# jthorborg/signalizer

Hardware: AMD Instinct MI355X
Metric: 32768-pt stereo STFT frames/sec (75% overlap); achieved HBM GB/s vs peak (higher is better)
Workload: dtype f32

## Files before the change

signalizer_amd/build.py:

```python
from __future__ import annotations

import os
import subprocess
import sys

HERE = os.path.dirname(os.path.abspath(__file__))
CSRC = os.path.join(HERE, "csrc")
LIB = os.path.join(HERE, "libsgz.so")
SOURCES = ["plan.cpp", "spectrum_fft.hip", "spectrum_real.hip", "spectrum_generic.hip", "spectrum_post.hip", "resonator.hip", "scope_vector.hip", "scope_dense.hip", "scope_stream.hip", "vector_stream.hip", "sharded.hip", "tracker.hip", "api.hip", "realtime.hip", "line_graph.hip", "view_translate.hip", "image_resize.hip", "ring_resize.hip", "spectrum_present.hip", "pcm.hip", "overview.hip", "overview_stats.hip", "overview_power.hip", "overview_cross.hip", "overview_flux.hip", "overview_pct.hip", "wave_columns.hip", "level_columns.hip", "truepeak_columns.hip", "loudness_columns.hip", "field_columns.hip", "band_columns.hip", "hist_columns.hip", "run_columns.hip"]
DRIVER = os.path.join(HERE, "librtdriver.so")
DRIVER_SRC = os.path.join(os.path.dirname(HERE), "tools", "rt_driver.cpp")
HEADERS = ["plan.hpp", "rt_lockfree.hpp", "kernels.hpp", "fft_common.hpp", "fft_scalar.hpp", "chunk_map.hpp", "real_common.hpp", "late_fix.hpp", "stft_body.hpp", "complex_dc.hpp", "decay_body.hpp", "runtime.hpp", "rt_common.hpp", "trace.hpp", "fade_chain.hpp", "scope_ring.hpp", "order_key.hpp", "column_lanes.hpp", "overview_kinds.hpp", os.path.join("..", "..", "include", "sgz.h")]


def _hipcc() -> str:
    for c in (os.environ.get("HIPCC"), "/opt/rocm/bin/hipcc", "hipcc"):
        if c and (os.path.isabs(c) and os.path.exists(c) or not os.path.isabs(c)):
            return c
    return "hipcc"


def stale() -> bool:
    if not os.path.exists(LIB):
        return True
# ... 7 lines not shown
        return LIB
    srcs = [os.path.join(CSRC, f) for f in SOURCES if os.path.exists(os.path.join(CSRC, f))]
    objs = []
    os.makedirs(os.path.join(HERE, "build"), exist_ok=True)
    procs = []
    for s in srcs:
        o = os.path.join(HERE, "build", os.path.basename(s) + ".o")
        objs.append(o)
        if s.endswith(".cpp"):
            cmd = [_hipcc(), "-O2", "-std=c++17", "-fPIC", "-ffp-contract=off", "-x", "c++", "-c", s, "-o", o]
        else:
            cmd = [_hipcc(), "--offload-arch=gfx950", "-O3", "-std=c++17", "-fPIC", "-fhip-fp32-correctly-rounded-divide-sqrt",
                   "-x", "hip", "-c", s, "-o", o] + os.environ.get("SGZ_EXTRA_HIPCC_FLAGS", "").split()
            if s.endswith(("spectrum_fft.hip", "spectrum_real.hip", "resonator.hip")):
                cmd.append("-fno-slp-vectorize")
        if verbose:
            print(" ".join(cmd))
        procs.append((s, subprocess.Popen(cmd, stdout=subprocess.PIPE, stderr=subprocess.STDOUT)))
    for s, p in procs:
        out, _ = p.communicate()
        if p.returncode != 0:
            sys.stderr.write(out.decode(errors="replace"))
            raise RuntimeError(f"hipcc failed on {s}")
    cmd = [_hipcc(), "--offload-arch=gfx950", "-shared", "-fPIC", "-o", LIB] + objs + ["-ldl"]
    subprocess.check_call(cmd)
    build_driver()
    return LIB



# ... 15 lines not shown
```

signalizer_amd/csrc/real_common.hpp:

```cpp
#pragma once
#include "chunk_map.hpp"
#include "fft_scalar.hpp"

namespace sgz {

struct ChannelIndex {
    int n, off;
    __device__ __forceinline__ int size() const { return n; }
    __device__ __forceinline__ int operator()(int k) const { return chunkPos(k - off); }
    __device__ __forceinline__ bool holds(int k) const { return k >= off && k <= off + n / 2; }
};

constexpr int realXFloats(int M) { return (chunkPos(M) + 1 + 16 + 1) & ~1; }

constexpr int kTw2Row = 34 * 2, kTw2Floats = 32 * kTw2Row;
constexpr size_t realExtraFloats(uint32_t maxSlots, uint32_t T, bool tw2InLds)
{
    const size_t a = size_t(maxSlots) + 1 + T, b = tw2InLds ? kTw2Floats + 4 : 0;
    return a > b ? a : b;
}

__device__ __forceinline__ float realBinMag(v2 a, v2 b, v2 w)
{
    const float ex = a.x + b.x, ey = a.y - b.y;
    const float dx = a.x - b.x, dy = a.y + b.y;
    const float xr = ex + (w.x * dy + w.y * dx);
    const float xi = ey + (w.y * dy - w.x * dx);
    return __builtin_amdgcn_sqrtf(xr * xr + xi * xi);
}

struct UnitId { int side, pair; uint32_t task, frame, self; };
template <bool MONO, typename P>
__device__ __forceinline__ UnitId unitOfIndex(const P &prm, uint32_t unit, const uint32_t nb, const bool mates = false)
{
    const uint32_t rs = prm.roundSize;
    if (nb >= 64u && rs >= 8u && (rs & 7u) == 0u) {
        const uint32_t base = (unit / rs) * rs;
        const uint32_t nbr = nb - base < rs ? nb - base : rs;
        const uint32_t x = (unit - base) & 7u;
        uint32_t i = (unit - base) >> 3;
        const uint32_t per = nbr >> 3, extra = nbr & 7u;
        if (mates) {
            const uint32_t c = rs >> 4, n = per + (x < extra ? 1u : 0u);
            if ((rs & 15u) == 0u && n > c && n <= 2u * c) {
                const uint32_t k = n - c;
                i = i < k ? 2u * i : i >= c ? 2u * (i - c) + 1u : i + k;
            }
        }
        unit = base + x * per + (x < extra ? x : extra) + i;
    }
    UnitId u;
    u.side = MONO ? 0 : int(unit & 1u);
    uint32_t task = MONO ? unit : unit >> 1;
    u.frame = task; u.pair = 0;
    if (prm.C > 1u) { const uint32_t F = uint32_t(prm.frames), pr = task / F, fr = task - pr * F; task = fr * prm.C + pr; u.frame = fr; u.pair = int(pr); }
    u.task = task;
    u.self = (task << 1) | uint32_t(u.side);
    return u;
}

template <bool MONO>
__device__ __forceinline__ UnitId unitOf(const RealParams &prm) { return unitOfIndex<MONO>(prm, blockIdx.x, gridDim.x); }

typedef const RealParams __attribute__((address_space(4))) WalkParams;
__device__ __forceinline__ WalkParams *walkParams()
{
    WalkParams *p = (WalkParams *)__builtin_amdgcn_kernarg_segment_ptr();
    asm volatile("" : "+s"(p));
    return p;
}
template <bool WALK> struct ParamsOf {
    typedef const RealParams T;
    static __device__ __forceinline__ T *get(const RealParams &launch) { return &launch; }
};
template <> struct ParamsOf<true> {
    typedef WalkParams T;
    static __device__ __forceinline__ T *get(const RealParams &) { return walkParams(); }
};

inline hipError_t grantLds(const void *kernel, size_t need, size_t (&granted)[64])
{
    int dev = 0;
    hipError_t e = hipGetDevice(&dev);
    if (e != hipSuccess) return e;
    if (dev >= 0 && dev < 64 && granted[dev] >= need) return hipSuccess;
    e = hipFuncSetAttribute(kernel, hipFuncAttributeMaxDynamicSharedMemorySize, int(need));
    if (e == hipSuccess && dev >= 0 && dev < 64) granted[dev] = need;
    return e;
}

}
```

signalizer_amd/csrc/spectrum_post.hip:

```cpp
#include <hip/hip_runtime.h>
#include <stdint.h>

#include <type_traits>

#include "decay_body.hpp"

namespace sgz {

__global__ void __launch_bounds__(256) decayLocalKernel(const DecayParams prm)
{
    const size_t perChunk = size_t(prm.C) * prm.sides * prm.P;
    const size_t gid = size_t(blockIdx.x) * blockDim.x + threadIdx.x;
    if (gid >= perChunk * prm.numChunks) return;
    const uint32_t chunk = uint32_t(gid / perChunk);
    const size_t rem = gid - size_t(chunk) * perChunk;
    const uint32_t pixel = uint32_t(rem % prm.P);
    const uint32_t ps = uint32_t(rem / prm.P);
    const uint32_t pair = ps / prm.sides, side = ps - pair * prm.sides;

    float a[G];
#pragma unroll
    for (int k = 0; k < G; ++k) {
        const size_t si = ((size_t(pair) * G + k) * prm.P + pixel) * 2 + side;
        a[k] = (chunk == 0 && prm.stateIn) ? prm.stateIn[si] : 0.f;
// ... 138 lines not shown
{
    for (;;) {
        uint32_t seen;
        asm volatile("ds_read_b32 %0, %1\n\ts_waitcnt lgkmcnt(0)" : "=v"(seen) : "v"(progressAddr) : "memory");
        if (seen >= chunk) break;
        __builtin_amdgcn_s_sleep(1);
    }
}

__device__ __forceinline__ uint32_t pixelGroup()
{
    const uint32_t b = blockIdx.x, n = gridDim.x;
    return (n & 7u) == 0 ? (b & 7u) * (n >> 3) + (b >> 3) : b;
}

template <int PX>
__global__ void __launch_bounds__(1024) decayColourFusedKernel(const DecayParams prm)
{
    __shared__ float aggS[kFusedChunks][PX];
    __shared__ float carryS[kFusedChunks][PX];
    __shared__ float magS[kFusedChunks * kMaxChunk][PX];
    __shared__ uint32_t progress;
    __shared__ double logTab[16][2];
    stageLogfTable(logTab);
    const uint32_t progressAddr = uint32_t(uintptr_t((__attribute__((address_space(3))) const void *)&progress));
    if (threadIdx.x == 0) progress = 0;
    const uint32_t tid = threadIdx.x;
    const size_t perFrame = size_t(prm.C) * prm.sides * prm.P;
    const float pole = prm.sc.pole[0];
    const uint32_t items = uint32_t(prm.frames) * PX;
    {
        constexpr int ROUNDS = kFusedChunks * kMaxChunk * PX / 1024;
        float m[ROUNDS], nyRe[ROUNDS], nyIm[ROUNDS], best[ROUNDS];
        const bool lateGroup = prm.hasLate && pixelGroup() * PX + PX > prm.late.fixFrom0;
#pragma unroll
        for (int r = 0; r < ROUNDS; ++r) {
            const uint32_t e = tid + 1024u * r, px = e % PX, f = e / PX;
            const uint32_t pixel = pixelGroup() * PX + px;
            const bool in = e < items && pixel < prm.P;
            m[r] = in ? prm.mapped[size_t(f) * perFrame + pixel] : 0.f;
            nyRe[r] = nyIm[r] = 0.f; best[r] = __builtin_inff();
            if (lateGroup && in && pixel >= prm.late.fixFrom0) {
                nyRe[r] = prm.late.ny[2 * size_t(f)]; nyIm[r] = prm.late.ny[2 * size_t(f) + 1];
                best[r] = lateBestSquare(prm.late, long(f), 0, pixel);
            }
        }
#pragma unroll
        for (int r = 0; r < ROUNDS; ++r) {
            const uint32_t e = tid + 1024u * r, px = e % PX, f = e / PX;
            const uint32_t pixel = pixelGroup() * PX + px;
            float v = m[r] * prm.magScale;
            if (lateGroup && e < items && pixel >= prm.late.fixFrom0 && pixel < prm.P)
                v = lateNyquistPixel(prm.late, lateNyquistValue(prm.late, nyRe[r], nyIm[r]), best[r], v);
            magS[f][px] = v;
        }
    }
    __syncthreads();
    static_assert(64 % PX == 0 && 960 % PX == 0, "thread tid's items tid - 64 + 960 k are all of pixel tid % PX");
    const uint32_t px = tid % PX;
    const uint32_t pixel = pixelGroup() * PX + px;
    if (tid < kFusedChunks * PX) {
// ... 565 lines not shown
    }
    if (prm.rgba && live && pl < len) reinterpret_cast<uchar4 *>(prm.rgba)[size_t(f0 + pl) * prm.P + pixel] = toRgba8(cb);
}

hipError_t launchDecayEmit(const DecayParams &prm, hipStream_t stream)
{
    const uint32_t firstChunk = (prm.rgba || prm.lines) ? 0u : prm.numChunks - 1;
    const unsigned grid = unsigned(size_t((prm.P + 31) / 32) * (prm.numChunks - firstChunk));
    static_assert(kMaxChunk == 8, "decayEmitPairsKernel: 8 frames x 32 pixels = one workgroup");
    if (prm.C >= 2) hipLaunchKernelGGL(decayEmitPairsKernel, dim3(grid), dim3(256), 0, stream, prm, firstChunk);
    else hipLaunchKernelGGL(decayEmitKernel, dim3(grid), dim3(256), 0, stream, prm, firstChunk);
    return hipGetLastError();
}

}
```

signalizer_amd/csrc/spectrum_real.hip:

```cpp
#include <algorithm>

#include "real_common.hpp"

#ifdef SGZ_DEBUG
#define RCLK(slot)                                                                                                     \
    do {                                                                                                               \
        if (prm.phaseClock && (tid & 63) == 0 && unit == long(prm.clkUnit)) prm.phaseClock[16 * (tid >> 6) + (slot)] = __builtin_readcyclecounter(); \
    } while (0)
#define RTRACE(which)                                                                                                  \
    do {                                                                                                               \
        if (prm.phaseClock && prm.clkUnit == 0xffffu && tid == 0) {                                                    \
            unsigned long long *t = prm.phaseClock + 256 + 4 * unit;                                                   \
            t[which] = __builtin_amdgcn_s_memrealtime();                                                               \
            if (which == 0) { t[2] = __builtin_amdgcn_s_getreg(4 | (31 << 11)); t[3] = __builtin_amdgcn_s_getreg(20 | (31 << 11)) | (static_cast<unsigned long long>(blockIdx.x) << 32); } \
        }                                                                                                              \
    } while (0)
#else
#define RCLK(slot) do { } while (0)
#define RTRACE(which) do { } while (0)
#endif

namespace sgz {

template <int R1, int LR1, int BASE, int Q = 0>
__device__ __forceinline__ void e1WriteRun(uint32_t wa, const v2 (&c)[32])
{
    if constexpr (Q < R1) { ldsWrite64<(Q & 15) * 512 * 8>(wa + uint32_t(Q >> 4) * 65536u, c[BASE + brev(Q, LR1)]); e1WriteRun<R1, LR1, BASE, Q + 1>(wa, c); }
}

template <int R1, int LR1, int Q = 0>
__device__ __forceinline__ void e1WritePairRun(uint32_t wa, const v2 (&c)[32])
{
    if constexpr (Q < R1) { ldsWrite128<(Q & 15) * 512 * 8>(wa + uint32_t(Q >> 4) * 65536u, c[brev(Q, LR1)], c[R1 + brev(Q, LR1)]); e1WritePairRun<R1, LR1, Q + 1>(wa, c); }
}
// ... 26 lines not shown

__device__ __forceinline__ void windowPairCos(v2 &lo, v2 &hi, const int a32, const v2 pc, const v2 ps, const v2 p0)
{
    v2 t = pc;
    if (a32 != 0) {
        const v2 k = v2{cos32(a32), sin32(a32)};
        v2 m;
        asm("v_pk_mul_f32 %0, %1, %2 op_sel:[0,1] op_sel_hi:[1,1]" : "=v"(m) : "v"(ps), "s"(k));
        asm("v_pk_fma_f32 %0, %1, %2, %3 op_sel:[0,0,0] op_sel_hi:[1,0,1] neg_lo:[0,0,1] neg_hi:[0,0,1]" : "=v"(t) : "v"(pc), "s"(k), "v"(m));
    }
    v2 wa, wb;
    asm("v_pk_add_f32 %0, %1, %2" : "=v"(wa) : "v"(t), "s"(p0));
    asm("v_pk_add_f32 %0, %1, %2 neg_lo:[1,0] neg_hi:[1,0]" : "=v"(wb) : "v"(t), "s"(p0));
    lo = lo * wa;
    hi = hi * wb;
}

template <int LR1, int MIX, typename P>
__device__ __forceinline__ void realMapSettle(const P &prm, float *lds, const int tid, const int side, const long task, const long self,
                                              const ChunkTables &tb, ChunkMap<(1 << (LR1 + 5))> &mapper, float *re, float *ce, float *spec)
{
    constexpr int R = 32, R1 = 1 << LR1, T = R1 * R, M = R1 * R * R, N = 2 * M;
    constexpr bool MONO = MIX == 1 || MIX == 3;
    const ChannelIndex at{N, side ? M : 0};
    [[maybe_unused]] const long unit = MONO ? task : self;
    if (prm.binsOut) {
        float *dst = prm.binsOut + size_t(task) * (N + 1) + (side ? M : 0);
        for (int i = tid; i <= M; i += T)
            if (MONO || i != (side ? 0 : M)) dst[i] = lds[chunkPos(i)];
    }
// ... 10 lines not shown
                out[x] = complexDcPixel(prm.recsFull[x], prm.weights, prm.invSize, N, prm.mode,
                                        [&](int k) { return k >= N ? 0.f : lds[chunkPos(k)]; },
                                        [&](int sl) { return make_float2(spec[2 * sl], spec[2 * sl + 1]); });
            }
        }
        return;
    }
}

[[maybe_unused]] __device__ __forceinline__ void setWavePriority(const uint32_t p)
{
    if (p != 0u) { if (p == 1u) __builtin_amdgcn_s_setprio(1); else if (p == 2u) __builtin_amdgcn_s_setprio(2); else __builtin_amdgcn_s_setprio(3); }
}

constexpr uint32_t kNyHopRows = 4;
template <int LR1, bool PRIO, bool SHARE>
__device__ __forceinline__ void nyquistUnit(const RealParams &prm, float *lds, const uint32_t light, const int tid)
{
    constexpr int LR = 5, R = 32, R1 = 1 << LR1, RR = R * R;
    static_assert(LR1 == 4, "the Nyquist workgroups mirror the two-columns-per-thread form (N = 32768)");
    [[maybe_unused]] const long unit = 2 * long(light) + 1;
    RTRACE(0);
#ifdef SGZ_IMAGE_PRIO
    if constexpr (PRIO) setWavePriority(prm.prioNy);
#endif
#ifdef SGZ_SCHED_SWEEP
    for (uint32_t k = 0; k < prm.nyDelay; ++k) __builtin_amdgcn_s_sleep(16);
#endif
    const uint32_t F = prm.nyFrames, perPair = uint32_t(prm.frames) / F + (uint32_t(prm.frames) % F != 0u);
    const uint32_t pair = light / perPair, f0 = (light - pair * perPair) * F;
    const uint32_t f1 = f0 + F < uint32_t(prm.frames) ? f0 + F : uint32_t(prm.frames);
    const float *X0 = prm.planar + size_t(2 * pair + 1) * prm.chStride;
    const uint32_t lane16 = uint32_t(tid) * 16u;
    const float4 ph[2] = {ldg(prm.winPhase, lane16 * 2u), ldg(prm.winPhase + 1, lane16 * 2u)};
    const v2 p0 = v2{prm.winP0, prm.winP0};
    v2 *lds2 = reinterpret_cast<v2 *>(lds);
    auto columnSum = [&](v2 (&c)[R1], const int u) {
        const v2 pc = v2{ph[u].x, ph[u].y}, ps = v2{ph[u].z, ph[u].w};
#pragma unroll
        for (int j = 0; j < R1 / 2; ++j) windowPairCos(c[j], c[j + R1 / 2], j * (32 / R1), pc, ps, p0);
        ditPacked<LR1, 0>(c);
        lds2[2 * tid + u] = c[0];
    };
    auto tree2 = [&]() {
        if (tid < R) {
            v2 s[R];
#pragma unroll
            for (int h = 0; h < R; ++h) s[h] = lds2[tid + R * h];
            ditPacked<LR, 0>(s);
            lds2[RR + tid] = s[0];
        }
    };
    auto tree3 = [&](const uint32_t f) {
        if (tid == 0) {
            v2 s[R];
#pragma unroll
            for (int r = 0; r < R; ++r) s[r] = lds2[RR + r];
            const float4 *tab = prm.tw2Full;
#pragma unroll
            for (int i = 0; i < R / 4; ++i) {
                const float4 wa = tab[i], wb = tab[i + R / 4];
                if (i == 0) bflyPackedFusedTw<true>(s[0], s[R / 2], v2{1.f, 0.f}, v2{wb.x, wb.y});
                else bflyPackedFusedTw<false>(s[2 * i], s[2 * i + R / 2], v2{wa.x, wa.y}, v2{wb.x, wb.y});
                bflyPackedFusedTw<false>(s[2 * i + 1], s[2 * i + 1 + R / 2], v2{wa.z, wa.w}, v2{wb.z, wb.w});
            }
            ditPacked<LR, 0, R, 2>(s);
            prm.ny[((size_t(f) * prm.C + pair) << 1) | 1u] = 2.f * (s[0].x - s[0].y);
        }
    };
    constexpr uint32_t HOPROWS = kNyHopRows;
    if (SHARE && f1 - f0 > 1u && prm.hop == HOPROWS * 2u * uint32_t(RR)) {
        typedef float v4 __attribute__((ext_vector_type(4)));
        v4 raw[R1];
        {
            const float *X = X0 + size_t(f0) * prm.hop;
#pragma unroll
            for (int j = 0; j < R1; ++j) raw[j] = ldgPinned<v4>(X, uint32_t(RR * j) * 8u, lane16);
        }
        for (uint32_t f = f0; f < f1; ++f) {
#pragma unroll
            for (int u = 0; u < 2; ++u) {
                v2 c[R1];
#pragma unroll
                for (int j = 0; j < R1; ++j) c[j] = u ? v2{raw[j].z, raw[j].w} : v2{raw[j].x, raw[j].y};
                columnSum(c, u);
            }
            if (f + 1u < f1) {
                const float *X = X0 + size_t(f + 1u) * prm.hop;
#pragma unroll
                for (int j = 0; j < R1 - int(HOPROWS); ++j) raw[j] = raw[j + int(HOPROWS)];
#pragma unroll
                for (int j = R1 - int(HOPROWS); j < R1; ++j) raw[j] = ldgPinned<v4>(X, uint32_t(RR * j) * 8u, lane16);
            }
            constexpr int PARK = R1 - int(HOPROWS);
            v4 *park = reinterpret_cast<v4 *>(lds + 4 * RR) + (tid & 63);
            if (__builtin_amdgcn_readfirstlane(tid) < 64) {
                __syncthreads();
#pragma unroll
                for (int j = 0; j < PARK; ++j) park[64 * j] = raw[j];
                tree2();
                __syncthreads();
                tree3(f);
#pragma unroll
                for (int j = 0; j < PARK; ++j) raw[j] = park[64 * j];
            } else {
                __syncthreads();
                __syncthreads();
            }
        }
        RTRACE(1);
        return;
    }
    for (uint32_t f = f0; f < f1; ++f) {
        const float *X = X0 + size_t(f) * prm.hop;
#pragma unroll
        for (int u = 0; u < 2; ++u) {
            v2 c[R1];
#pragma unroll
            for (int j = 0; j < R1; ++j) c[j] = ldgPinned<v2>(X, uint32_t(RR * j) * 8u + 8u * u, lane16);
            columnSum(c, u);
        }
        __syncthreads();
        tree2();
        __syncthreads();
        tree3(f);
    }
    RTRACE(1);
}

template <int LR1, bool WCOS, int MIX = 0, bool PRIO = false>
__global__ void __launch_bounds__(1 << (LR1 + 5), 4) stftRealKernel(const RealParams launchPrm)
{
    constexpr int LR = 5, R = 32, R1 = 1 << LR1, T = R1 * R, RR = R * R, M = R1 * RR, N = 2 * M, U = R / R1;
    constexpr bool MONO = MIX == 1 || MIX == 3;
    constexpr bool SIDE0 = MIX == 4;
    constexpr bool mixed = MIX == 2 || MIX == 3;
    constexpr int PADSTRIDE = chunkPos(T);
    constexpr int ROW = R + 2, TILE = R * ROW;
    constexpr int XFLOATS = realXFloats(M);
    static_assert((T / R) * TILE <= XFLOATS, "the exchange-2 tiles end below the twiddle table");
    constexpr int TAB = (XFLOATS + 3) & ~3;
    extern __shared__ __attribute__((aligned(16))) float lds[];
    const int tid0 = threadIdx.x;

    constexpr bool WALK = LR1 == 5 && MIX == 0 && WCOS;
    const uint32_t heavyUnits = SIDE0 ? uint32_t(launchPrm.frames) * launchPrm.C : gridDim.x;
    if constexpr (SIDE0) {
        if (blockIdx.x >= heavyUnits) { nyquistUnit<LR1, PRIO, PRIO>(launchPrm, lds, blockIdx.x - heavyUnits, opaque(tid0)); return; }
    }
    const uint32_t totalUnits = WALK ? uint32_t(launchPrm.frames) * launchPrm.C * 2u : heavyUnits;
    uint32_t walkIndex = blockIdx.x;
    UnitId uid = unitOfIndex<MONO || SIDE0>(launchPrm, walkIndex, totalUnits, SIDE0 && launchPrm.mateAdjacent != 0u);
    [[maybe_unused]] bool firstUnit = true;
    [[maybe_unused]] uint32_t prioEarly = 0u, prioLate = 0u, prioEnds = 0u;
    if constexpr (LR1 == 4) {
        const uint32_t cus = launchPrm.roundSize >> 1;
#ifndef SGZ_STAGGER
#define SGZ_STAGGER 5
#endif
        if (cus && !launchPrm.pipelined && gridDim.x >= 2u * cus && blockIdx.x >= cus && blockIdx.x < 2u * cus) {
#pragma unroll
            for (int k = 0; k < SGZ_STAGGER; ++k) __builtin_amdgcn_s_sleep(32);
        }
#ifdef SGZ_SCHED_SWEEP
        else if (SIDE0 && blockIdx.x >= cus) {
            for (uint32_t k = 0; k < launchPrm.mateDelay; ++k) __builtin_amdgcn_s_sleep(16);
        }
#endif
#ifndef SGZ_NO_PRIO
        if (cus && !launchPrm.pipelined && gridDim.x > 2u * cus && gridDim.x <= 3u * cus) {
#else
        if (false) {
#endif
            const uint32_t generation = blockIdx.x / cus;
            if (generation == 0u) __builtin_amdgcn_s_setprio(2); else if (generation == 1u) __builtin_amdgcn_s_setprio(1); else __builtin_amdgcn_s_setprio(3);
        }
#ifdef SGZ_IMAGE_PRIO
        if constexpr (PRIO) {
#ifdef SGZ_SCHED_SWEEP
            const uint32_t rolePrio = blockIdx.x >= cus ? launchPrm.prioMate : blockIdx.x + cus < heavyUnits ? launchPrm.prioFirst : 0u;
            const uint32_t scope = launchPrm.prioScope;
#else
            const uint32_t rolePrio = blockIdx.x >= cus ? (launchPrm.prioMate ? uint32_t(SGZ_PRIO_MATE) : 0u)
                                                        : blockIdx.x + cus < heavyUnits ? (launchPrm.prioFirst ? uint32_t(SGZ_PRIO_FIRST) : 0u) : 0u;
            constexpr uint32_t scope = SGZ_PRIO_SCOPE;
#endif
            prioEarly = (scope == 0u || scope == 3u) ? rolePrio : 0u;
            prioLate = (scope == 1u || scope == 2u) ? rolePrio : 0u;
            prioEnds = (scope & 1u) ? rolePrio : 0u;
            prioEarly = __builtin_amdgcn_readfirstlane(prioEarly); prioLate = __builtin_amdgcn_readfirstlane(prioLate); prioEnds = __builtin_amdgcn_readfirstlane(prioEnds);
        }
#endif
    }
    constexpr bool PAIRED = U == 2;
    constexpr int COLSTEP = PAIRED ? 1 : T, COLLANE = PAIRED ? 2 : 1;
    constexpr bool FRONT = LR1 >= 4 && !mixed && WCOS;
#ifdef SGZ_DIET
    constexpr bool DIET = PAIRED && FRONT && LR1 == 4;
#else
    constexpr bool DIET = false;
#endif
    constexpr bool STREAM = LR1 == 4 && PAIRED && FRONT && !DIET;
    [[maybe_unused]] float4 phase[U];
    [[maybe_unused]] float2 twA[U], twB[U];
    [[maybe_unused]] float4 tw2piece, tw2tail;
    v2 c[R];
    for (;;) {
    typename ParamsOf<WALK>::T &prm = *ParamsOf<WALK>::get(launchPrm);
    auto samplesOf = [&](const UnitId &u) {
        const int firstCh = MONO ? (prm.mode == SGZ_CH_RIGHT ? 1 : 0) : (mixed ? 0 : u.side);
        return prm.planar + size_t(2 * u.pair + firstCh) * prm.chStride + size_t(u.frame) * prm.hop;
    };
    auto elemOf = [&](int e) { const int u = e / R1, j = e % R1; return (PAIRED ? u : T * u) + RR * j; };
    auto requestSamples = [&](const float *X, const int tid, auto partTag) {
        constexpr int part = decltype(partTag)::value;
        const uint32_t lane8 = uint32_t(tid) * (PAIRED ? 16u : 8u);
        if constexpr (PAIRED) {
            typedef float v4 __attribute__((ext_vector_type(4)));
#pragma unroll
            for (int i = 0; i < R1; ++i) {
                const int j = STREAM ? brev(i, LR1) : i;
                const v4 xv = ldgPinned<v4>(X, uint32_t(RR * j) * 8u, lane8); c[j] = v2{xv.x, xv.y}; c[R1 + j] = v2{xv.z, xv.w};
            }
        } else {
#pragma unroll
            for (int i = 0; i < R; ++i)
                if (part == 0 || ((i >> 3) & 1) == part - 1) c[i] = ldgPinned<v2>(X, uint32_t(elemOf(i)) * 8u, lane8);
        }
    };
    auto requestPhases = [&](const int tid) {
#pragma unroll
        for (int u = 0; u < (DIET ? 1 : U); ++u) phase[u] = ldg(prm.winPhase + COLSTEP * u, uint32_t(tid) * 16u * COLLANE);
    };
    auto requestTables = [&](const int tid) {
        if constexpr (FRONT) {
            if constexpr (WALK) tw2piece = prm.tw2Full[tid < kTw2Floats / 4 ? tid : 0];
            if constexpr (WCOS && !STREAM) requestPhases(tid);
#pragma unroll
// ... 5 lines not shown
            if (T < kTw2Floats / 4 && tid < kTw2Floats / 4 - T) tw2tail = prm.tw2Full[T + tid];
        }
    };
    if constexpr (WALK) {
        if (firstUnit) requestSamples(samplesOf(uid), tid0, std::integral_constant<int, 1>{});
        firstUnit = false;
    }
    const int tid = WALK ? opaque(tid0) : tid0;
    const int slot = tid >> 6, half = (tid >> 5) & 1, l = tid & 31, group = tid >> 5;
    const int q1 = half ? (slot == 0 ? R1 / 2 : R1 - slot) : slot;
    const int ix = half ? R - 1 - l : l;
    const uint32_t lane8 = uint32_t(tid) * (PAIRED ? 16u : 8u);
    [[maybe_unused]] const long unit = MONO ? long(uid.task) : long(uid.self);
    const int side = SIDE0 ? 0 : uid.side, pair = uid.pair;
    const long task = uid.task, frame = uid.frame, self = uid.self;

    const uint32_t maxSlots = prm.chunkSlots[0] > prm.chunkSlots[1] ? prm.chunkSlots[0] : prm.chunkSlots[1];
    const ChunkTables tb{prm.chunkEnds + side * T, prm.chunkReBase + side * T,
                         reinterpret_cast<const uint2 *>(prm.chunkRec) + size_t(side) * prm.P, prm.recs + size_t(side) * prm.P, prm.weights12,
                         prm.mapped ? prm.mapped + (size_t(task) * (MONO ? 1 : 2) + side) * prm.P : nullptr,
                         MONO ? nullptr : prm.nyBest + size_t(self) * 64, int(prm.fixFrom[side]), int(prm.P), side != 0,
#ifdef SGZ_DEBUG
                         (prm.phaseClock && unit == long(prm.clkUnit)) ? prm.phaseClock : nullptr};
#else
                         nullptr};
#endif
    const ChannelIndex at{N, side ? M : 0};
    float *re = lds + XFLOATS, *ce = re + maxSlots + 1;
    const int SCRATCH = XFLOATS + int(realExtraFloats(maxSlots, T, LR1 >= 4));
    float *spec = lds + SCRATCH + 2 * R;
// ... 1 lines not shown

    RCLK(0);
    RTRACE(0);
    if constexpr (LR1 >= 4 && !FRONT) {
        for (int i = tid; i < kTw2Floats / 4; i += T) reinterpret_cast<float4 *>(lds + TAB)[i] = prm.tw2Full[i];
    }
    {
        const float *X = samplesOf(uid);
        if constexpr (WALK) {
            requestTables(tid);
            __builtin_amdgcn_sched_barrier(0);
            requestSamples(X, tid, std::integral_constant<int, 2>{});
            __builtin_amdgcn_sched_barrier(0);
            if (tid < kTw2Floats / 4) reinterpret_cast<float4 *>(lds + TAB)[tid] = tw2piece;
        } else {
            if constexpr (STREAM) { requestPhases(tid); __builtin_amdgcn_sched_barrier(0); }
            requestSamples(X, tid, std::integral_constant<int, 0>{});
            requestTables(tid);
        }
        if constexpr (FRONT) __builtin_amdgcn_sched_barrier(0);
#ifdef SGZ_IMAGE_PRIO
        if constexpr (PRIO) setWavePriority(prioEarly);
#endif
        if (mixed) {
            const float *Y = X + prm.chStride;
            const float sgn = (MONO ? prm.mode == SGZ_CH_SIDE : side == 1) ? -1.f : 1.f;
            constexpr int YB = (LR1 == 5 || (PAIRED && !WCOS)) ? 4 : 8;
#pragma unroll
            for (int b0 = 0; b0 < R; b0 += YB) {
                float2 y[YB];
#pragma unroll
                for (int i = 0; i < YB; ++i) y[i] = ldg(reinterpret_cast<const float2 *>(Y) + elemOf(b0 + i), lane8);
#pragma unroll
// ... 331 lines not shown
            put(M, MONO ? fixB : 0.f);
        }
    }
    *reinterpret_cast<float2 *>(lds + chunkPos(32 * tid) + 32) = float2{0.f, 0.f};
    if (tid < 16) lds[chunkPos(M) + 1 + tid] = 0.f;
    ldsBarrier();
    RCLK(7);
    realMapSettle<LR1, MIX>(prm, lds, tid, side, task, self, tb, mapper, re, ce, spec);
    if constexpr (!WALK) break;
    else {
        if (!more) break;
        uid = nextUid;
        ldsBarrier();
    }
    }
}

template <int LR1>
__global__ void __launch_bounds__(1 << (LR1 + 5)) realMapFromBinsKernel(const RealParams prm)
{
    constexpr int R = 32, R1 = 1 << LR1, T = R1 * R, M = R1 * R * R, N = 2 * M;
    constexpr int XFLOATS = realXFloats(M);
    extern __shared__ __attribute__((aligned(16))) float lds[];
    const int tid = threadIdx.x;
    const long unit = blockIdx.x;
    const int side = int(unit & 1);
    const long task = unit >> 1;
    const long self = (task << 1) | side;
    const uint32_t maxSlots = prm.chunkSlots[0] > prm.chunkSlots[1] ? prm.chunkSlots[0] : prm.chunkSlots[1];
    const ChunkTables tb{prm.chunkEnds + side * T, prm.chunkReBase + side * T,
// ... 124 lines not shown
        if (N == 32768) e = wcos ? go(&stftRealKernel<4, true, 1>, 6, 512, 80 * 1024) : go(&stftRealKernel<4, false, 1>, 7, 512, 80 * 1024);
        else if (N == 16384) e = wcos ? go(&stftRealKernel<3, true, 1>, 8, 256, 40 * 1024) : go(&stftRealKernel<3, false, 1>, 9, 256, 40 * 1024);
        else if (N == 65536) e = wcos ? go(&stftRealKernel<5, true, 1>, 10, 1024, 160 * 1024) : go(&stftRealKernel<5, false, 1>, 11, 1024, 160 * 1024);
        else return hipErrorNotSupported;
        if (e != hipSuccess) return e;
        return hipGetLastError();
    }
    if (prm.mode == SGZ_CH_MIDSIDE) {
        if (N == 32768) e = wcos ? go(&stftRealKernel<4, true, 2>, 12, 512, 80 * 1024) : go(&stftRealKernel<4, false, 2>, 13, 512, 80 * 1024);
        else if (N == 16384) e = wcos ? go(&stftRealKernel<3, true, 2>, 14, 256, 40 * 1024) : go(&stftRealKernel<3, false, 2>, 15, 256, 40 * 1024);
        else if (N == 65536) e = wcos ? go(&stftRealKernel<5, true, 2>, 16, 1024, 160 * 1024) : go(&stftRealKernel<5, false, 2>, 17, 1024, 160 * 1024);
        else return hipErrorNotSupported;
        if (e != hipSuccess) return e;
        return hipGetLastError();
    }
#ifdef SGZ_IMAGE_PRIO
    if (side0 && ((prm.prioFirst | prm.prioMate | prm.prioNy) || (prm.nyFrames > 1u && prm.frames > 1 && prm.hop == kNyHopRows * 2048u)))
        e = go(&stftRealKernel<4, true, 4, true>, 28, 512, 80 * 1024);
    else
#endif
    if (side0) e = go(&stftRealKernel<4, true, 4>, 27, 512, 80 * 1024);
    else if (N == 32768) e = wcos ? go(&stftRealKernel<4, true>, 0, 512, 80 * 1024) : go(&stftRealKernel<4, false>, 1, 512, 80 * 1024);
    else if (N == 16384) e = wcos ? go(&stftRealKernel<3, true>, 4, 256, 40 * 1024) : go(&stftRealKernel<3, false>, 5, 256, 40 * 1024);
    else if (N == 65536) e = wcos ? go(&stftRealKernel<5, true>, 2, 1024, 160 * 1024) : go(&stftRealKernel<5, false>, 3, 1024, 160 * 1024);
    else return hipErrorNotSupported;
    if (e != hipSuccess) return e;
    return hipGetLastError();
}

}
```

Measured before the change: 14.94 million.

## Add front-entry STFT kernel with preloaded leading kernel arguments

Adds a new entry point for the side-0 real STFT kernel. The kernel takes a small front block of scalars (planar pointer, window phases, strides, hop, frames, round info) ahead of the full parameter struct, and the compiler is told to preload the leading kernel arguments into SGPRs. The first-round unit mapping, window-phase loads and sample requests can then be issued without waiting on kernarg loads from memory. Priority setup and other parameter reads are deferred until after the loads are in flight. This shortens the entry latency of each workgroup, at the cost of more template paths and a duplicated parameter copy per launch.

```diff
diff --git a/signalizer_amd/build.py b/signalizer_amd/build.py
--- a/signalizer_amd/build.py
+++ b/signalizer_amd/build.py
@@ -8,6 +8,7 @@
 CSRC = os.path.join(HERE, "csrc")
 LIB = os.path.join(HERE, "libsgz.so")
 SOURCES = ["plan.cpp", "spectrum_fft.hip", "spectrum_real.hip", "spectrum_generic.hip", "spectrum_post.hip", "resonator.hip", "scope_vector.hip", "scope_dense.hip", "scope_stream.hip", "vector_stream.hip", "sharded.hip", "tracker.hip", "api.hip", "realtime.hip", "line_graph.hip", "view_translate.hip", "image_resize.hip", "ring_resize.hip", "spectrum_present.hip", "pcm.hip", "overview.hip", "overview_stats.hip", "overview_power.hip", "overview_cross.hip", "overview_flux.hip", "overview_pct.hip", "wave_columns.hip", "level_columns.hip", "truepeak_columns.hip", "loudness_columns.hip", "field_columns.hip", "band_columns.hip", "hist_columns.hip", "run_columns.hip"]
+PRELOAD_FLAGS = ["-mllvm", "-amdgpu-kernarg-preload-count=12"]
 DRIVER = os.path.join(HERE, "librtdriver.so")
 DRIVER_SRC = os.path.join(os.path.dirname(HERE), "tools", "rt_driver.cpp")
 HEADERS = ["plan.hpp", "rt_lockfree.hpp", "kernels.hpp", "fft_common.hpp", "fft_scalar.hpp", "chunk_map.hpp", "real_common.hpp", "late_fix.hpp", "stft_body.hpp", "complex_dc.hpp", "decay_body.hpp", "runtime.hpp", "rt_common.hpp", "trace.hpp", "fade_chain.hpp", "scope_ring.hpp", "order_key.hpp", "column_lanes.hpp", "overview_kinds.hpp", os.path.join("..", "..", "include", "sgz.h")]
@@ -45,6 +46,8 @@
                    "-x", "hip", "-c", s, "-o", o] + os.environ.get("SGZ_EXTRA_HIPCC_FLAGS", "").split()
             if s.endswith(("spectrum_fft.hip", "spectrum_real.hip", "resonator.hip")):
                 cmd.append("-fno-slp-vectorize")
+            if s.endswith("spectrum_real.hip"):
+                cmd += PRELOAD_FLAGS
         if verbose:
             print(" ".join(cmd))
         procs.append((s, subprocess.Popen(cmd, stdout=subprocess.PIPE, stderr=subprocess.STDOUT)))
diff --git a/signalizer_amd/csrc/real_common.hpp b/signalizer_amd/csrc/real_common.hpp
--- a/signalizer_amd/csrc/real_common.hpp
+++ b/signalizer_amd/csrc/real_common.hpp
@@ -30,12 +30,12 @@
 }
 
 struct UnitId { int side, pair; uint32_t task, frame, self; };
-template <bool MONO, typename P>
+template <bool MONO, typename P, bool FIRSTROUND = false>
 __device__ __forceinline__ UnitId unitOfIndex(const P &prm, uint32_t unit, const uint32_t nb, const bool mates = false)
 {
     const uint32_t rs = prm.roundSize;
     if (nb >= 64u && rs >= 8u && (rs & 7u) == 0u) {
-        const uint32_t base = (unit / rs) * rs;
+        const uint32_t base = (FIRSTROUND && unit < rs) ? 0u : (unit / rs) * rs;
         const uint32_t nbr = nb - base < rs ? nb - base : rs;
         const uint32_t x = (unit - base) & 7u;
         uint32_t i = (unit - base) >> 3;
@@ -59,6 +59,15 @@
     return u;
 }
 
+struct RealFront {
+    const float *planar; const float4 *winPhase;
+    uint32_t chStrideLo, chStrideHi;
+    uint32_t hop, frames, C, roundSize, nyFrames;
+    uint32_t flags;
+    __device__ __forceinline__ size_t chStride() const { return (size_t(chStrideHi) << 32) | chStrideLo; }
+};
+constexpr uint32_t kFrontMates = 1u, kFrontLateSecond = 2u;
+
 template <bool MONO>
 __device__ __forceinline__ UnitId unitOf(const RealParams &prm) { return unitOfIndex<MONO>(prm, blockIdx.x, gridDim.x); }
 
@@ -69,13 +78,28 @@
     asm volatile("" : "+s"(p));
     return p;
 }
-template <bool WALK> struct ParamsOf {
+__device__ __forceinline__ WalkParams *frontBlock()
+{
+    static_assert(sizeof(RealFront) == 48 && alignof(RealParams) == 8, "the block's offset in a front entry's argument segment");
+    return (WalkParams *)((const char __attribute__((address_space(4))) *)__builtin_amdgcn_kernarg_segment_ptr() + sizeof(RealFront));
+}
+__device__ __forceinline__ WalkParams *frontParams()
+{
+    WalkParams *p = frontBlock();
+    asm volatile("" : "+s"(p));
+    return p;
+}
+template <bool WALK, bool EARLY = false> struct ParamsOf {
     typedef const RealParams T;
     static __device__ __forceinline__ T *get(const RealParams &launch) { return &launch; }
 };
-template <> struct ParamsOf<true> {
+template <> struct ParamsOf<true, false> {
     typedef WalkParams T;
     static __device__ __forceinline__ T *get(const RealParams &) { return walkParams(); }
+};
+template <> struct ParamsOf<false, true> {
+    typedef WalkParams T;
+    static __device__ __forceinline__ T *get(const RealParams &) { return frontParams(); }
 };
 
 inline hipError_t grantLds(const void *kernel, size_t need, size_t (&granted)[64])
diff --git a/signalizer_amd/csrc/spectrum_post.hip b/signalizer_amd/csrc/spectrum_post.hip
--- a/signalizer_amd/csrc/spectrum_post.hip
+++ b/signalizer_amd/csrc/spectrum_post.hip
@@ -176,9 +176,17 @@
     return (n & 7u) == 0 ? (b & 7u) * (n >> 3) + (b >> 3) : b;
 }
 
+#ifdef SGZ_DEBUG
+__device__ unsigned long long *g_kbEntryClock;
+#define KB_STAMP(name) const unsigned long long name = __builtin_readcyclecounter()
+#else
+#define KB_STAMP(name) do { } while (0)
+#endif
+
 template <int PX>
 __global__ void __launch_bounds__(1024) decayColourFusedKernel(const DecayParams prm)
 {
+    KB_STAMP(clkEntry);
     __shared__ float aggS[kFusedChunks][PX];
     __shared__ float carryS[kFusedChunks][PX];
     __shared__ float magS[kFusedChunks * kMaxChunk][PX];
@@ -191,6 +199,10 @@
     const size_t perFrame = size_t(prm.C) * prm.sides * prm.P;
     const float pole = prm.sc.pole[0];
     const uint32_t items = uint32_t(prm.frames) * PX;
+#ifdef SGZ_DEBUG
+    __builtin_amdgcn_sched_barrier(0);
+#endif
+    KB_STAMP(clkFront);
     {
         constexpr int ROUNDS = kFusedChunks * kMaxChunk * PX / 1024;
         float m[ROUNDS], nyRe[ROUNDS], nyIm[ROUNDS], best[ROUNDS];
@@ -207,6 +219,14 @@
                 best[r] = lateBestSquare(prm.late, long(f), 0, pixel);
             }
         }
+#ifdef SGZ_DEBUG
+        __builtin_amdgcn_sched_barrier(0);
+        KB_STAMP(clkRequested);
+        if (g_kbEntryClock && tid == 0) {
+            unsigned long long *t = g_kbEntryClock + 4 * blockIdx.x;
+            t[0] = clkEntry; t[1] = clkFront; t[2] = clkRequested; t[3] = blockIdx.x;
+        }
+#endif
 #pragma unroll
         for (int r = 0; r < ROUNDS; ++r) {
             const uint32_t e = tid + 1024u * r, px = e % PX, f = e / PX;
@@ -802,3 +822,10 @@
 }
 
 }
+
+#ifdef SGZ_DEBUG
+extern "C" int sgz_debug_kb_entry_clocks(unsigned long long *d_clocks)
+{
+    return int(hipMemcpyToSymbol(HIP_SYMBOL(sgz::g_kbEntryClock), &d_clocks, sizeof d_clocks));
+}
+#endif
diff --git a/signalizer_amd/csrc/spectrum_real.hip b/signalizer_amd/csrc/spectrum_real.hip
--- a/signalizer_amd/csrc/spectrum_real.hip
+++ b/signalizer_amd/csrc/spectrum_real.hip
@@ -3,21 +3,35 @@
 #include "real_common.hpp"
 
 #ifdef SGZ_DEBUG
+template <typename T> __device__ __forceinline__ T &blockOf(T &x) { return x; }
+template <typename T> __device__ __forceinline__ T &blockOf(T *x) { return *x; }
 #define RCLK(slot)                                                                                                     \
     do {                                                                                                               \
-        if (prm.phaseClock && (tid & 63) == 0 && unit == long(prm.clkUnit)) prm.phaseClock[16 * (tid >> 6) + (slot)] = __builtin_readcyclecounter(); \
+        if (blockOf(prm).phaseClock && (tid & 63) == 0 && unit == long(blockOf(prm).clkUnit)) blockOf(prm).phaseClock[16 * (tid >> 6) + (slot)] = __builtin_readcyclecounter(); \
     } while (0)
 #define RTRACE(which)                                                                                                  \
     do {                                                                                                               \
-        if (prm.phaseClock && prm.clkUnit == 0xffffu && tid == 0) {                                                    \
-            unsigned long long *t = prm.phaseClock + 256 + 4 * unit;                                                   \
+        if (blockOf(prm).phaseClock && blockOf(prm).clkUnit == 0xffffu && tid == 0) {                                                    \
+            unsigned long long *t = blockOf(prm).phaseClock + 256 + 4 * unit;                                                   \
             t[which] = __builtin_amdgcn_s_memrealtime();                                                               \
             if (which == 0) { t[2] = __builtin_amdgcn_s_getreg(4 | (31 << 11)); t[3] = __builtin_amdgcn_s_getreg(20 | (31 << 11)) | (static_cast<unsigned long long>(blockIdx.x) << 32); } \
         }                                                                                                              \
     } while (0)
+#define RENTRY(t0, t1, t2)                                                                                             \
+    do {                                                                                                               \
+        if (blockOf(prm).phaseClock && blockOf(prm).clkUnit == 0xfffeu && tid == 0) {                                                    \
+            unsigned long long *t = blockOf(prm).phaseClock + 256 + 4 * unit;                                                   \
+            t[0] = (t0); t[1] = (t1); t[2] = (t2); t[3] = blockIdx.x;                                                  \
+        }                                                                                                              \
+    } while (0)
+#define RSTAMP(name) const unsigned long long name = __builtin_readcyclecounter()
+#define RMARK(name) name = __builtin_readcyclecounter()
 #else
 #define RCLK(slot) do { } while (0)
 #define RTRACE(which) do { } while (0)
+#define RENTRY(t0, t1, t2) do { } while (0)
+#define RSTAMP(name) do { } while (0)
+#define RMARK(name) do { } while (0)
 #endif
 
 namespace sgz {
@@ -74,6 +88,18 @@
     asm("v_pk_add_f32 %0, %1, %2 neg_lo:[1,0] neg_hi:[1,0]" : "=v"(wb) : "v"(t), "s"(p0));
     lo = lo * wa;
     hi = hi * wb;
+}
+
+template <int LR1, bool BYARRIVAL>
+__device__ __forceinline__ void requestRowPairs(v2 (&c)[32], const float *X, const uint32_t lane16)
+{
+    constexpr int R1 = 1 << LR1, RR = 32 * 32;
+    typedef float v4 __attribute__((ext_vector_type(4)));
+#pragma unroll
+    for (int i = 0; i < R1; ++i) {
+        const int j = BYARRIVAL ? brev(i, LR1) : i;
+        const v4 xv = ldgPinned<v4>(X, uint32_t(RR * j) * 8u, lane16); c[j] = v2{xv.x, xv.y}; c[R1 + j] = v2{xv.z, xv.w};
+    }
 }
 
 template <int LR1, int MIX, typename P>
@@ -114,28 +140,46 @@
 }
 
 constexpr uint32_t kNyHopRows = 4;
-template <int LR1, bool PRIO, bool SHARE>
-__device__ __forceinline__ void nyquistUnit(const RealParams &prm, float *lds, const uint32_t light, const int tid)
+template <int LR1, bool PRIO, bool SHARE, bool EARLY = false, typename P>
+__device__ __forceinline__ void nyquistUnit(P &block, float *lds, const uint32_t light, const int tid,
+                                            [[maybe_unused]] const RealFront &front, [[maybe_unused]] const unsigned long long clkEntry = 0)
 {
     constexpr int LR = 5, R = 32, R1 = 1 << LR1, RR = R * R;
+    P *prm = &block;
     static_assert(LR1 == 4, "the Nyquist workgroups mirror the two-columns-per-thread form (N = 32768)");
     [[maybe_unused]] const long unit = 2 * long(light) + 1;
     RTRACE(0);
+    [[maybe_unused]] auto settlePriority = [&]() __attribute__((always_inline)) {
 #ifdef SGZ_IMAGE_PRIO
-    if constexpr (PRIO) setWavePriority(prm.prioNy);
-#endif
+        if constexpr (PRIO) setWavePriority(prm->prioNy);
+#endif
+    };
+    if constexpr (!EARLY) {
+        settlePriority();
 #ifdef SGZ_SCHED_SWEEP
-    for (uint32_t k = 0; k < prm.nyDelay; ++k) __builtin_amdgcn_s_sleep(16);
-#endif
-    const uint32_t F = prm.nyFrames, perPair = uint32_t(prm.frames) / F + (uint32_t(prm.frames) % F != 0u);
-    const uint32_t pair = light / perPair, f0 = (light - pair * perPair) * F;
-    const uint32_t f1 = f0 + F < uint32_t(prm.frames) ? f0 + F : uint32_t(prm.frames);
-    const float *X0 = prm.planar + size_t(2 * pair + 1) * prm.chStride;
+        for (uint32_t k = 0; k < prm->nyDelay; ++k) __builtin_amdgcn_s_sleep(16);
+#endif
+    }
+    const uint32_t frames = EARLY ? front.frames : uint32_t(prm->frames), hop = EARLY ? front.hop : prm->hop;
+    const uint32_t F = EARLY ? front.nyFrames : prm->nyFrames;
+    uint32_t pair = 0u, f0 = light * F;
+    if (!EARLY || front.C != 1u) {
+        const uint32_t perPair = frames / F + (frames % F != 0u);
+        pair = light / perPair; f0 = (light - pair * perPair) * F;
+    }
+    const uint32_t f1 = f0 + F < frames ? f0 + F : frames;
+    const float *X0 = EARLY ? front.planar + size_t(2 * pair + 1) * front.chStride()
+                            : prm->planar + size_t(2 * pair + 1) * prm->chStride;
     const uint32_t lane16 = uint32_t(tid) * 16u;
-    const float4 ph[2] = {ldg(prm.winPhase, lane16 * 2u), ldg(prm.winPhase + 1, lane16 * 2u)};
-    const v2 p0 = v2{prm.winP0, prm.winP0};
+    const float4 *const winPhase = EARLY ? front.winPhase : prm->winPhase;
+    const float4 ph[2] = {ldg(winPhase, lane16 * 2u), ldg(winPhase + 1, lane16 * 2u)};
+#ifdef SGZ_DEBUG
+    __builtin_amdgcn_sched_barrier(0);
+    RSTAMP(clkPhases);
+#endif
     v2 *lds2 = reinterpret_cast<v2 *>(lds);
     auto columnSum = [&](v2 (&c)[R1], const int u) {
+        const v2 p0 = v2{prm->winP0, prm->winP0};
         const v2 pc = v2{ph[u].x, ph[u].y}, ps = v2{ph[u].z, ph[u].w};
 #pragma unroll
         for (int j = 0; j < R1 / 2; ++j) windowPairCos(c[j], c[j + R1 / 2], j * (32 / R1), pc, ps, p0);
@@ -156,7 +200,7 @@
             v2 s[R];
 #pragma unroll
             for (int r = 0; r < R; ++r) s[r] = lds2[RR + r];
-            const float4 *tab = prm.tw2Full;
+            const float4 *tab = prm->tw2Full;
 #pragma unroll
             for (int i = 0; i < R / 4; ++i) {
                 const float4 wa = tab[i], wb = tab[i + R / 4];
@@ -165,18 +209,20 @@
                 bflyPackedFusedTw<false>(s[2 * i + 1], s[2 * i + 1 + R / 2], v2{wa.z, wa.w}, v2{wb.z, wb.w});
             }
             ditPacked<LR, 0, R, 2>(s);
-            prm.ny[((size_t(f) * prm.C + pair) << 1) | 1u] = 2.f * (s[0].x - s[0].y);
+            prm->ny[((size_t(f) * prm->C + pair) << 1) | 1u] = 2.f * (s[0].x - s[0].y);
         }
     };
     constexpr uint32_t HOPROWS = kNyHopRows;
-    if (SHARE && f1 - f0 > 1u && prm.hop == HOPROWS * 2u * uint32_t(RR)) {
+    if (SHARE && f1 - f0 > 1u && hop == HOPROWS * 2u * uint32_t(RR)) {
         typedef float v4 __attribute__((ext_vector_type(4)));
         v4 raw[R1];
         {
-            const float *X = X0 + size_t(f0) * prm.hop;
+            const float *X = X0 + size_t(f0) * hop;
 #pragma unroll
             for (int j = 0; j < R1; ++j) raw[j] = ldgPinned<v4>(X, uint32_t(RR * j) * 8u, lane16);
         }
+        if constexpr (EARLY) { __builtin_amdgcn_sched_barrier(0); asm volatile("" : "+s"(prm)); settlePriority(); }
+        RENTRY(clkEntry, clkPhases, 0ull);
         for (uint32_t f = f0; f < f1; ++f) {
 #pragma unroll
             for (int u = 0; u < 2; ++u) {
@@ -186,7 +232,7 @@
                 columnSum(c, u);
             }
             if (f + 1u < f1) {
-                const float *X = X0 + size_t(f + 1u) * prm.hop;
+                const float *X = X0 + size_t(f + 1u) * hop;
 #pragma unroll
                 for (int j = 0; j < R1 - int(HOPROWS); ++j) raw[j] = raw[j + int(HOPROWS)];
 #pragma unroll
@@ -211,8 +257,10 @@
         RTRACE(1);
         return;
     }
+    if constexpr (EARLY) { __builtin_amdgcn_sched_barrier(0); asm volatile("" : "+s"(prm)); settlePriority(); }
+    RENTRY(clkEntry, clkPhases, 0ull);
     for (uint32_t f = f0; f < f1; ++f) {
-        const float *X = X0 + size_t(f) * prm.hop;
+        const float *X = X0 + size_t(f) * hop;
 #pragma unroll
         for (int u = 0; u < 2; ++u) {
             v2 c[R1];
@@ -228,9 +276,10 @@
     RTRACE(1);
 }
 
-template <int LR1, bool WCOS, int MIX = 0, bool PRIO = false>
-__global__ void __launch_bounds__(1 << (LR1 + 5), 4) stftRealKernel(const RealParams launchPrm)
-{
+template <int LR1, bool WCOS, int MIX, bool PRIO, bool EARLY>
+__device__ __forceinline__ void stftRealBody(const RealParams &launchPrm, [[maybe_unused]] const RealFront &front)
+{
+    RSTAMP(clkEntry);
     constexpr int LR = 5, R = 32, R1 = 1 << LR1, T = R1 * R, RR = R * R, M = R1 * RR, N = 2 * M, U = R / R1;
     constexpr bool MONO = MIX == 1 || MIX == 3;
     constexpr bool SIDE0 = MIX == 4;
@@ -244,29 +293,44 @@
     const int tid0 = threadIdx.x;
 
     constexpr bool WALK = LR1 == 5 && MIX == 0 && WCOS;
-    const uint32_t heavyUnits = SIDE0 ? uint32_t(launchPrm.frames) * launchPrm.C : gridDim.x;
+    static_assert(!EARLY || !WALK, "the WALK kernel's block is its only parameter");
+    const uint32_t heavyUnits = SIDE0 ? (EARLY ? front.frames * front.C : uint32_t(launchPrm.frames) * launchPrm.C) : gridDim.x;
     if constexpr (SIDE0) {
-        if (blockIdx.x >= heavyUnits) { nyquistUnit<LR1, PRIO, PRIO>(launchPrm, lds, blockIdx.x - heavyUnits, opaque(tid0)); return; }
+        if (blockIdx.x >= heavyUnits) {
+#ifdef SGZ_DEBUG
+            const unsigned long long clkLaunch = clkEntry;
+#else
+            const unsigned long long clkLaunch = 0;
+#endif
+            if constexpr (EARLY) nyquistUnit<LR1, PRIO, PRIO, true>(*frontBlock(), lds, blockIdx.x - heavyUnits, opaque(tid0), front, clkLaunch);
+            else nyquistUnit<LR1, PRIO, PRIO, false>(launchPrm, lds, blockIdx.x - heavyUnits, opaque(tid0), front, clkLaunch);
+            return;
+        }
     }
     const uint32_t totalUnits = WALK ? uint32_t(launchPrm.frames) * launchPrm.C * 2u : heavyUnits;
     uint32_t walkIndex = blockIdx.x;
-    UnitId uid = unitOfIndex<MONO || SIDE0>(launchPrm, walkIndex, totalUnits, SIDE0 && launchPrm.mateAdjacent != 0u);
+    UnitId uid;
+    if constexpr (EARLY) uid = unitOfIndex<MONO || SIDE0, RealFront, true>(front, walkIndex, totalUnits, SIDE0 && (front.flags & kFrontMates) != 0u);
+    else uid = unitOfIndex<MONO || SIDE0>(launchPrm, walkIndex, totalUnits, SIDE0 && launchPrm.mateAdjacent != 0u);
     [[maybe_unused]] bool firstUnit = true;
     [[maybe_unused]] uint32_t prioEarly = 0u, prioLate = 0u, prioEnds = 0u;
+    [[maybe_unused]] const uint32_t cus = (EARLY ? front.roundSize : launchPrm.roundSize) >> 1;
     if constexpr (LR1 == 4) {
-        const uint32_t cus = launchPrm.roundSize >> 1;
 #ifndef SGZ_STAGGER
 #define SGZ_STAGGER 5
 #endif
-        if (cus && !launchPrm.pipelined && gridDim.x >= 2u * cus && blockIdx.x >= cus && blockIdx.x < 2u * cus) {
+        if (EARLY ? ((front.flags & kFrontLateSecond) != 0u && blockIdx.x >= cus && blockIdx.x < 2u * cus)
+                  : (cus && !launchPrm.pipelined && gridDim.x >= 2u * cus && blockIdx.x >= cus && blockIdx.x < 2u * cus)) {
 #pragma unroll
             for (int k = 0; k < SGZ_STAGGER; ++k) __builtin_amdgcn_s_sleep(32);
         }
 #ifdef SGZ_SCHED_SWEEP
-        else if (SIDE0 && blockIdx.x >= cus) {
+        else if (!EARLY && SIDE0 && blockIdx.x >= cus) {
             for (uint32_t k = 0; k < launchPrm.mateDelay; ++k) __builtin_amdgcn_s_sleep(16);
         }
 #endif
+    }
+    [[maybe_unused]] auto settlePriorities = [&](const auto &launchPrm) __attribute__((always_inline)) {
 #ifndef SGZ_NO_PRIO
         if (cus && !launchPrm.pipelined && gridDim.x > 2u * cus && gridDim.x <= 3u * cus) {
 #else
@@ -291,7 +355,8 @@
             prioEarly = __builtin_amdgcn_readfirstlane(prioEarly); prioLate = __builtin_amdgcn_readfirstlane(prioLate); prioEnds = __builtin_amdgcn_readfirstlane(prioEnds);
         }
 #endif
-    }
+    };
+    if constexpr (LR1 == 4 && !EARLY) settlePriorities(launchPrm);
     constexpr bool PAIRED = U == 2;
     constexpr int COLSTEP = PAIRED ? 1 : T, COLLANE = PAIRED ? 2 : 1;
     constexpr bool FRONT = LR1 >= 4 && !mixed && WCOS;
@@ -305,8 +370,22 @@
     [[maybe_unused]] float2 twA[U], twB[U];
     [[maybe_unused]] float4 tw2piece, tw2tail;
     v2 c[R];
+#ifdef SGZ_DEBUG
+    [[maybe_unused]] unsigned long long clkPhases = 0, clkSamples = 0;
+#endif
+    if constexpr (EARLY) {
+        static_assert(STREAM, "a front entry requests as the streamed load phase does");
+#pragma unroll
+        for (int u = 0; u < U; ++u) phase[u] = ldg(front.winPhase + COLSTEP * u, uint32_t(tid0) * 16u * COLLANE);
+        __builtin_amdgcn_sched_barrier(0);
+        RMARK(clkPhases);
+        requestRowPairs<LR1, true>(c, front.planar + size_t(2 * uid.pair + uid.side) * front.chStride() + size_t(uid.frame) * front.hop,
+                                   uint32_t(tid0) * 16u);
+        __builtin_amdgcn_sched_barrier(0);
+        RMARK(clkSamples);
+    }
     for (;;) {
-    typename ParamsOf<WALK>::T &prm = *ParamsOf<WALK>::get(launchPrm);
+    typename ParamsOf<WALK, EARLY>::T &prm = *ParamsOf<WALK, EARLY>::get(launchPrm);
     auto samplesOf = [&](const UnitId &u) {
         const int firstCh = MONO ? (prm.mode == SGZ_CH_RIGHT ? 1 : 0) : (mixed ? 0 : u.side);
         return prm.planar + size_t(2 * u.pair + firstCh) * prm.chStride + size_t(u.frame) * prm.hop;
@@ -316,12 +395,7 @@
         constexpr int part = decltype(partTag)::value;
         const uint32_t lane8 = uint32_t(tid) * (PAIRED ? 16u : 8u);
         if constexpr (PAIRED) {
-            typedef float v4 __attribute__((ext_vector_type(4)));
-#pragma unroll
-            for (int i = 0; i < R1; ++i) {
-                const int j = STREAM ? brev(i, LR1) : i;
-                const v4 xv = ldgPinned<v4>(X, uint32_t(RR * j) * 8u, lane8); c[j] = v2{xv.x, xv.y}; c[R1 + j] = v2{xv.z, xv.w};
-            }
+            requestRowPairs<LR1, STREAM>(c, X, lane8);
         } else {
 #pragma unroll
             for (int i = 0; i < R; ++i)
@@ -357,6 +431,7 @@
     [[maybe_unused]] const long unit = MONO ? long(uid.task) : long(uid.self);
     const int side = SIDE0 ? 0 : uid.side, pair = uid.pair;
     const long task = uid.task, frame = uid.frame, self = uid.self;
+    if constexpr (EARLY && LR1 == 4) settlePriorities(prm);
 
     const uint32_t maxSlots = prm.chunkSlots[0] > prm.chunkSlots[1] ? prm.chunkSlots[0] : prm.chunkSlots[1];
     const ChunkTables tb{prm.chunkEnds + side * T, prm.chunkReBase + side * T,
@@ -388,9 +463,20 @@
             __builtin_amdgcn_sched_barrier(0);
             if (tid < kTw2Floats / 4) reinterpret_cast<float4 *>(lds + TAB)[tid] = tw2piece;
         } else {
-            if constexpr (STREAM) { requestPhases(tid); __builtin_amdgcn_sched_barrier(0); }
-            requestSamples(X, tid, std::integral_constant<int, 0>{});
+            if constexpr (!EARLY) {
+                if constexpr (STREAM) { requestPhases(tid); __builtin_amdgcn_sched_barrier(0); }
+                RMARK(clkPhases);
+                requestSamples(X, tid, std::integral_constant<int, 0>{});
+#ifdef SGZ_DEBUG
+                __builtin_amdgcn_sched_barrier(0);
+#endif
+                RMARK(clkSamples);
+            }
             requestTables(tid);
+#ifdef SGZ_DEBUG
+            __builtin_amdgcn_sched_barrier(0);
+            RENTRY(clkEntry, clkPhases, clkSamples);
+#endif
         }
         if constexpr (FRONT) __builtin_amdgcn_sched_barrier(0);
 #ifdef SGZ_IMAGE_PRIO
@@ -752,6 +838,20 @@
         ldsBarrier();
     }
     }
+}
+
+template <int LR1, bool WCOS, int MIX = 0, bool PRIO = false>
+__global__ void __launch_bounds__(1 << (LR1 + 5), 4) stftRealKernel(const RealParams launchPrm)
+{
+    stftRealBody<LR1, WCOS, MIX, PRIO, false>(launchPrm, RealFront{});
+}
+template <int LR1, bool WCOS, int MIX, bool PRIO>
+__global__ void __launch_bounds__(1 << (LR1 + 5), 4)
+stftRealKernelFront(const float *planar, const float4 *winPhase, const uint32_t chStrideLo, const uint32_t chStrideHi, const uint32_t hop,
+                    const uint32_t frames, const uint32_t C, const uint32_t roundSize, const uint32_t nyFrames, const uint32_t flags,
+                    const RealParams launchPrm)
+{
+    stftRealBody<LR1, WCOS, MIX, PRIO, true>(launchPrm, RealFront{planar, winPhase, chStrideLo, chStrideHi, hop, frames, C, roundSize, nyFrames, flags});
 }
 
 template <int LR1>
@@ -906,12 +1006,21 @@
         if (e != hipSuccess) return e;
         return hipGetLastError();
     }
+    auto goFront = [&](auto kern, int slot) -> hipError_t {
+        if (ldsBytes > 80 * 1024 || prm.frames > 0x7fffffffL) return hipErrorInvalidValue;
+        if (hipError_t e = grantLds(reinterpret_cast<const void *>(kern), ldsBytes, granted[slot]); e != hipSuccess) return e;
+        const uint32_t cus = prm.roundSize >> 1;
+        const uint32_t flags = (prm.mateAdjacent ? kFrontMates : 0u) | (cus && !prm.pipelined && units >= 2 * long(cus) ? kFrontLateSecond : 0u);
+        hipLaunchKernelGGL(kern, dim3(unsigned(units)), dim3(512), ldsBytes, stream, prm.planar, prm.winPhase, uint32_t(prm.chStride),
+                           uint32_t(uint64_t(prm.chStride) >> 32), prm.hop, uint32_t(prm.frames), prm.C, prm.roundSize, prm.nyFrames, flags, prm);
+        return hipSuccess;
+    };
 #ifdef SGZ_IMAGE_PRIO
     if (side0 && ((prm.prioFirst | prm.prioMate | prm.prioNy) || (prm.nyFrames > 1u && prm.frames > 1 && prm.hop == kNyHopRows * 2048u)))
-        e = go(&stftRealKernel<4, true, 4, true>, 28, 512, 80 * 1024);
+        e = goFront(&stftRealKernelFront<4, true, 4, true>, 28);
     else
 #endif
-    if (side0) e = go(&stftRealKernel<4, true, 4>, 27, 512, 80 * 1024);
+    if (side0) e = goFront(&stftRealKernelFront<4, true, 4, false>, 27);
     else if (N == 32768) e = wcos ? go(&stftRealKernel<4, true>, 0, 512, 80 * 1024) : go(&stftRealKernel<4, false>, 1, 512, 80 * 1024);
     else if (N == 16384) e = wcos ? go(&stftRealKernel<3, true>, 4, 256, 40 * 1024) : go(&stftRealKernel<3, false>, 5, 256, 40 * 1024);
     else if (N == 65536) e = wcos ? go(&stftRealKernel<5, true>, 2, 1024, 160 * 1024) : go(&stftRealKernel<5, false>, 3, 1024, 160 * 1024);
```

New measurement: 14.94 million. Within noise of the previous version (-0.0%).
